# ucsdmanorlab/PSSR2

Measured on AMD Instinct MI355X. Metric: HR tiles/sec (512^2 4xSR) train, higher is better.
Workload: dtype bf16

## Files before the change

include/pssr_mi355.h:

```cpp
#ifndef PSSR_MI355_H
#define PSSR_MI355_H

#include <stdint.h>

#ifdef __cplusplus
extern "C" {
#endif

typedef void* pssr_stream_t;

enum { PSSR_F32 = 0, PSSR_BF16 = 1, PSSR_F16 = 2 };

enum {
    PSSR_OK = 0,
    PSSR_ERR_ARG = -1,
    PSSR_ERR_LAUNCH = -2,
    PSSR_ERR_UNSUPPORTED = -3
};

int pssr_abi_version(void);
const char* pssr_last_error(void);

int pssr_pack_conv_weight(const float* w_oihw, void* packed, int cout, int cin, int ks,
                          int ci_begin, int ci_count, int mode, const int32_t* n_perm,
// ... 25 lines not shown
#define PSSR_STAT_STRIPES 32
#define PSSR_STAT_ROWS (2 * PSSR_STAT_STRIPES)

enum {
    PSSR_FLAG_RELU = 1,
    PSSR_FLAG_STATS = 2,
    PSSR_FLAG_HEADQ = 8,
    PSSR_FLAG_AFFINE = 4,
    PSSR_FLAG_SOLO = 32,
    PSSR_FLAG_SHUF2 = 16
};

typedef struct pssr_conv_desc {
    int32_t dtype;
    int32_t n, h, w;
    const void* in0; int32_t in0_cstride, in0_coff, cin0, taps0;
    const void* w0;
    const void* in1; int32_t in1_cstride, in1_coff, cin1, taps1;
    const void* w1;
    int32_t prologue;
    const float* pro_scale;
    const float* pro_shift;
    void* out; int32_t out_cstride, out_coff, cout, n_pad;
    const float* bias;
    int32_t epilogue, flags;
    const void* aux; int32_t aux_cstride, aux_coff;
    const float* aux_scale; const float* aux_shift;
    const float* aux_mean; const float* aux_invstd;
    double* stats;
    int32_t in0_blk, out_blk, aux_blk;
    float out_scale, out_shift;
    void* workspace; int64_t workspace_bytes;
    const float* head_w; float* head_q;
} pssr_conv_desc;

int pssr_conv2d(const pssr_conv_desc* desc, pssr_stream_t stream);
int64_t pssr_conv2d_workspace_bytes(const pssr_conv_desc* desc);
int pssr_conv2d_pipeline_mode(int mode);

int pssr_set_option(const char* name, int value);
int pssr_get_option(const char* name);

typedef struct pssr_wgrad_desc {
    int32_t dtype;
    int32_t n, h, w;
    const void* dy; int32_t dy_cstride, dy_coff, dy_blk, cout;
    const void* in; int32_t in_cstride, in_coff, in_blk, cin_pad;
    int32_t taps;
    int32_t prologue; const float* pro_scale; const float* pro_shift;
    float* dw;
    int32_t dw_parts;
} pssr_wgrad_desc;

int pssr_conv2d_wgrad(const pssr_wgrad_desc* desc, pssr_stream_t stream);
int pssr_conv2d_wgrad_parts(const pssr_wgrad_desc* desc);



int pssr_channel_stats_nchw(const float* x, int n, int c, int64_t hw, float pre_scale, float pre_shift,
                            double* stats, pssr_stream_t stream);

int pssr_bn_finalize(const double* stats, double count, const float* gamma, const float* beta, float eps,
                     float momentum, float* running_mean, float* running_var, float* scale, float* shift,
                     float* mean, float* invstd, int c, pssr_stream_t stream);
int pssr_bn_eval_affine(const float* gamma, const float* beta, const float* running_mean,
                        const float* running_var, float eps, float* scale, float* shift, int c,
                        pssr_stream_t stream);
int pssr_bn_relu_apply(const void* y, int y_cs, int y_co, const float* scale, const float* shift, void* a, int a_cs,
                       int a_co, int64_t npix, int c, int dtype, pssr_stream_t stream);
// ... 270 lines not shown
```

pssr2_amd/_lib.py:

```python
from __future__ import annotations

import ctypes as C
import os
from pathlib import Path

_LIB_PATH = Path(__file__).resolve().parent / "libpssr_mi355.so"
_lib = None

F32, BF16, F16 = 0, 1, 2
PRO_NONE, PRO_BN_RELU, PRO_GELU = 0, 1, 2
EPI_STORE, EPI_TAIL, EPI_DGRAD_MASK, EPI_FINAL, EPI_DGRAD_GELU, EPI_HEADQ = 0, 1, 2, 3, 4, 5
FLAG_RELU, FLAG_STATS, FLAG_AFFINE, FLAG_HEADQ, FLAG_SHUF2, FLAG_SOLO = 1, 2, 4, 8, 16, 32

c_void_p, c_int, c_i64, c_float = C.c_void_p, C.c_int, C.c_int64, C.c_float


class ConvDesc(C.Structure):
    _fields_ = [
        ("dtype", C.c_int32), ("n", C.c_int32), ("h", C.c_int32), ("w", C.c_int32),
        ("in0", c_void_p), ("in0_cstride", C.c_int32), ("in0_coff", C.c_int32), ("cin0", C.c_int32), ("taps0", C.c_int32),
        ("w0", c_void_p),
        ("in1", c_void_p), ("in1_cstride", C.c_int32), ("in1_coff", C.c_int32), ("cin1", C.c_int32), ("taps1", C.c_int32),
        ("w1", c_void_p),
        ("prologue", C.c_int32), ("pro_scale", c_void_p), ("pro_shift", c_void_p),
        ("out", c_void_p), ("out_cstride", C.c_int32), ("out_coff", C.c_int32), ("cout", C.c_int32), ("n_pad", C.c_int32),
        ("bias", c_void_p),
        ("epilogue", C.c_int32), ("flags", C.c_int32),
        ("aux", c_void_p), ("aux_cstride", C.c_int32), ("aux_coff", C.c_int32),
        ("aux_scale", c_void_p), ("aux_shift", c_void_p), ("aux_mean", c_void_p), ("aux_invstd", c_void_p),
        ("stats", c_void_p),
        ("in0_blk", C.c_int32), ("out_blk", C.c_int32), ("aux_blk", C.c_int32),
        ("out_scale", C.c_float), ("out_shift", C.c_float),
        ("workspace", c_void_p), ("workspace_bytes", C.c_int64),
        ("head_w", c_void_p), ("head_q", c_void_p),
    ]


class WgradDesc(C.Structure):
    _fields_ = [
        ("dtype", C.c_int32), ("n", C.c_int32), ("h", C.c_int32), ("w", C.c_int32),
        ("dy", c_void_p), ("dy_cstride", C.c_int32), ("dy_coff", C.c_int32), ("dy_blk", C.c_int32), ("cout", C.c_int32),
        ("in_", c_void_p), ("in_cstride", C.c_int32), ("in_coff", C.c_int32), ("in_blk", C.c_int32), ("cin_pad", C.c_int32),
        ("taps", C.c_int32),
        ("prologue", C.c_int32), ("pro_scale", c_void_p), ("pro_shift", c_void_p),
        ("dw", c_void_p), ("dw_parts", C.c_int32),
    ]


class GatherItem(C.Structure):
    _fields_ = [("src", C.c_void_p), ("sh", C.c_int), ("sw", C.c_int), ("rot", C.c_int), ("flip_axis", C.c_int)]


class SheetDesc(C.Structure):
    _fields_ = [("base", C.c_void_p), ("frames", C.c_int), ("h", C.c_int), ("w", C.c_int), ("reserved", C.c_int)]


class WindowItem(C.Structure):
    _fields_ = [("sheet", C.c_int), ("frame0", C.c_int), ("y0", C.c_int), ("x0", C.c_int), ("rot", C.c_int), ("flip_axis", C.c_int)]


class CollagePanel(C.Structure):
    _fields_ = [("src", C.c_void_p), ("image_stride", C.c_int64), ("row_pitch", C.c_int32), ("src_h", C.c_int32), ("src_w", C.c_int32),
                ("is_f32", C.c_int32), ("yi", C.c_void_p), ("xi", C.c_void_p)]


COPY_BATCH_MAX = 16

# ... 64 lines not shown
```

pssr2_amd/csrc/conv_igemm.hip:

```cpp
#include "conv_igemm_args.h"

using pssr_conv::ConvArgs;

extern "C" int pssr_conv2d_pipeline_mode(int mode) {
    (void)mode;
    return 0;
}

static int conv2d_entry(const pssr_conv_desc* d, pssr_stream_t stream, long* query_ws);

#ifdef PSSR_V3_STAMPS
static unsigned* g_stamp_buf = nullptr;
extern "C" void pssr_debug_stamp_buffer(void* p) { g_stamp_buf = (unsigned*)p; }
#endif

extern "C" int pssr_conv2d(const pssr_conv_desc* d, pssr_stream_t stream) { return conv2d_entry(d, stream, nullptr); }

extern "C" int64_t pssr_conv2d_workspace_bytes(const pssr_conv_desc* d) {
    long bytes = 0;
    const int rc = conv2d_entry(d, nullptr, &bytes);
    return rc != PSSR_OK ? (int64_t)rc : (int64_t)bytes;
}

static int conv2d_entry(const pssr_conv_desc* d, pssr_stream_t stream, long* query_ws) {
    PSSR_CHECK(d != nullptr, PSSR_ERR_ARG, "conv2d: null desc");
    PSSR_CHECK(d->dtype == PSSR_F32 || d->dtype == PSSR_BF16 || d->dtype == PSSR_F16, PSSR_ERR_ARG, "conv2d: bad dtype %d", d->dtype);
    const int kch = d->dtype == PSSR_F32 ? 8 : 16;
    const int esz = d->dtype == PSSR_F32 ? 4 : 2;
    PSSR_CHECK(d->n > 0 && d->h > 0 && d->w > 0, PSSR_ERR_ARG, "conv2d: bad shape %dx%dx%d", d->n, d->h, d->w);
    PSSR_CHECK(query_ws || (d->in0 && d->w0 && d->out), PSSR_ERR_ARG, "conv2d: null pointer");
    PSSR_CHECK(d->cin0 > 0 && d->cin0 % kch == 0, PSSR_ERR_ARG, "conv2d: cin0=%d must be a positive multiple of %d", d->cin0, kch);
    PSSR_CHECK(d->taps0 == 9 || d->taps0 == 1, PSSR_ERR_ARG, "conv2d: taps0=%d", d->taps0);
    PSSR_CHECK((d->in0_cstride * esz) % 16 == 0 && (d->in0_coff * esz) % 16 == 0, PSSR_ERR_ARG, "conv2d: in0 stride/offset not 16-byte aligned");
    PSSR_CHECK(d->in0_coff + d->cin0 <= d->in0_cstride, PSSR_ERR_ARG, "conv2d: in0 slice exceeds stride");
    if (d->cin1) {
        PSSR_CHECK(d->in1 && d->w1 && d->cin1 % kch == 0 && d->taps1 == 1, PSSR_ERR_ARG, "conv2d: source 1 must be a 1x1 (or flat-K) source");
        PSSR_CHECK((d->in1_cstride * esz) % 16 == 0 && (d->in1_coff * esz) % 16 == 0 && d->in1_coff + d->cin1 <= d->in1_cstride, PSSR_ERR_ARG, "conv2d: in1 stride/offset");
    }
    if (d->epilogue == PSSR_EPI_FINAL) {
        PSSR_CHECK(d->cout > 0 && d->cout <= 32 && (d->flags & ~PSSR_FLAG_SOLO) == 0, PSSR_ERR_ARG, "conv2d: EPI_FINAL needs 0 < cout <= 32 and no flags");
    } else {
        PSSR_CHECK(d->cout > 0 && d->cout % 4 == 0, PSSR_ERR_ARG, "conv2d: cout=%d must be a positive multiple of 4", d->cout);
        PSSR_CHECK(d->out_coff % 4 == 0 && d->out_cstride % 4 == 0 &&
                   d->out_coff + ((d->flags & PSSR_FLAG_SHUF2) ? d->cout / 4 : d->cout) <= d->out_cstride, PSSR_ERR_ARG, "conv2d: out stride/offset");
    }
    PSSR_CHECK(d->n_pad % 128 == 0 && d->n_pad >= d->cout, PSSR_ERR_ARG, "conv2d: n_pad=%d", d->n_pad);
    PSSR_CHECK(d->prologue >= 0 && d->prologue <= PSSR_PRO_GELU, PSSR_ERR_ARG, "conv2d: prologue=%d", d->prologue);
    PSSR_CHECK(d->prologue != PSSR_PRO_BN_RELU || (d->pro_scale && d->pro_shift), PSSR_ERR_ARG, "conv2d: prologue needs scale/shift");
    PSSR_CHECK(d->epilogue >= 0 && d->epilogue <= 5, PSSR_ERR_ARG, "conv2d: epilogue=%d", d->epilogue);
    if (d->flags & PSSR_FLAG_HEADQ)
        PSSR_CHECK(d->epilogue == PSSR_EPI_STORE && !(d->flags & (PSSR_FLAG_STATS | PSSR_FLAG_AFFINE)) && (d->flags & PSSR_FLAG_RELU), PSSR_ERR_ARG,
                   "conv2d: FLAG_HEADQ goes with EPI_STORE | FLAG_RELU only");
    if (d->epilogue == PSSR_EPI_HEADQ || (d->flags & PSSR_FLAG_HEADQ)) {
        PSSR_CHECK(query_ws || (d->head_w && d->head_q), PSSR_ERR_ARG, "conv2d: EPI_HEADQ needs head_w / head_q");
        PSSR_CHECK(esz == 2 && d->cout == 1024 && d->taps0 == 9 && d->w >= 16 && d->h >= 16 && d->prologue != PSSR_PRO_GELU && !(d->flags & PSSR_FLAG_STATS),
                   PSSR_ERR_UNSUPPORTED, "conv2d: EPI_HEADQ needs 16-bit storage, a 3x3 source, cout = 16 x 64 (4 x upscaling) and at least 16x16 pixels");
    }
    PSSR_CHECK(d->in0_blk >= 0 && d->out_blk >= 0 && d->aux_blk >= 0 && d->in0_blk <= 3 && d->out_blk <= 3 && d->aux_blk <= 3, PSSR_ERR_ARG, "conv2d: blocked order");
    {
        const int mb = d->in0_blk > d->out_blk ? (d->in0_blk > d->aux_blk ? d->in0_blk : d->aux_blk) : (d->out_blk > d->aux_blk ? d->out_blk : d->aux_blk);
        PSSR_CHECK(d->h % (1 << mb) == 0 && d->w % (1 << mb) == 0, PSSR_ERR_ARG, "conv2d: blocked order needs H,W multiples of r");
    }
    if (d->epilogue == PSSR_EPI_TAIL || d->epilogue == PSSR_EPI_DGRAD_MASK) {
        PSSR_CHECK(d->aux && d->aux_scale && d->aux_shift && d->aux_coff % 4 == 0 && d->aux_cstride % 4 == 0, PSSR_ERR_ARG, "conv2d: epilogue needs aux tensor");
    }
    if (d->epilogue == PSSR_EPI_DGRAD_GELU)
        PSSR_CHECK(d->aux && d->aux_coff % 4 == 0 && d->aux_cstride % 4 == 0, PSSR_ERR_ARG, "conv2d: GELU backward needs the pre-activation as aux");
    if (d->flags & PSSR_FLAG_SHUF2) {
        PSSR_CHECK(d->epilogue == PSSR_EPI_STORE && !(d->flags & (PSSR_FLAG_STATS | PSSR_FLAG_HEADQ)) && d->out_blk == 0, PSSR_ERR_ARG,
                   "conv2d: FLAG_SHUF2 goes with EPI_STORE, without statistics, tap planes or a blocked output order");
        PSSR_CHECK(esz == 2 && d->cout % 32 == 0 && d->out_coff % 8 == 0 && d->out_cstride % 8 == 0 && pssr_tunables().conv_epi8, PSSR_ERR_UNSUPPORTED,
                   "conv2d: FLAG_SHUF2 needs 16-bit storage, cout a multiple of 32 and 8-channel aligned outputs");
    }
    if (d->flags & PSSR_FLAG_AFFINE) {
        PSSR_CHECK(d->epilogue == PSSR_EPI_STORE && !(d->flags & PSSR_FLAG_STATS) && d->aux_scale && d->aux_shift, PSSR_ERR_ARG,
                   "conv2d: FLAG_AFFINE needs EPI_STORE without statistics and aux_scale / aux_shift");
        PSSR_CHECK(esz == 2 && d->cout % 8 == 0 && d->out_coff % 8 == 0 && d->out_cstride % 8 == 0 && pssr_tunables().conv_epi8, PSSR_ERR_UNSUPPORTED,
                   "conv2d: FLAG_AFFINE needs 16-bit storage and 8-channel aligned outputs");
    }
    if (d->flags & PSSR_FLAG_STATS) {
        PSSR_CHECK(d->stats != nullptr, PSSR_ERR_ARG, "conv2d: stats buffer missing");
        PSSR_CHECK(d->epilogue != PSSR_EPI_DGRAD_MASK || (d->aux_mean && d->aux_invstd), PSSR_ERR_ARG, "conv2d: mask stats need mean/invstd");
        PSSR_CHECK(d->epilogue != PSSR_EPI_TAIL, PSSR_ERR_ARG, "conv2d: no stats on tail");
    }
    ConvArgs a;
    a.N = d->n; a.H = d->h; a.W = d->w;
    a.in[0] = d->in0; a.in_cs[0] = d->in0_cstride; a.in_co[0] = d->in0_coff; a.nchunks[0] = d->cin0 / kch; a.taps[0] = d->taps0; a.w[0] = d->w0;
    a.in[1] = d->in1; a.in_cs[1] = d->in1_cstride; a.in_co[1] = d->in1_coff; a.nchunks[1] = d->cin1 ? d->cin1 / kch : 0; a.taps[1] = d->cin1 ? d->taps1 : 1; a.w[1] = d->w1;
    a.prologue = d->prologue; a.pro_scale = d->pro_scale; a.pro_shift = d->pro_shift;
    a.out = d->out; a.out_cs = d->out_cstride; a.out_co = d->out_coff; a.cout = d->cout; a.n_pad = d->n_pad;
    a.bias = d->bias; a.epi = d->epilogue; a.flags = d->flags;
    a.aux = d->aux; a.aux_cs = d->aux_cstride; a.aux_co = d->aux_coff;
    a.aux_scale = d->aux_scale; a.aux_shift = d->aux_shift; a.aux_mean = d->aux_mean; a.aux_invstd = d->aux_invstd;
    a.stats = d->stats;
    a.in0_blk = d->in0_blk; a.out_blk = d->out_blk; a.aux_blk = d->aux_blk;
    a.out_scale = d->out_scale; a.out_shift = d->out_shift;
    const bool headq = a.epi == PSSR_EPI_HEADQ || (a.flags & PSSR_FLAG_HEADQ);
    a.head_w = headq ? d->head_w : nullptr;
    a.head_q = headq ? d->head_q : nullptr;
    a.tiles_x = a.tiles_y = a.tiles_n = 0;
    a.epi8 = esz == 2 && d->epilogue != PSSR_EPI_FINAL && d->cout % 8 == 0 && d->out_coff % 8 == 0 && d->out_cstride % 8 == 0 &&
             (d->epilogue == PSSR_EPI_STORE || d->epilogue == PSSR_EPI_HEADQ || (d->aux_coff % 8 == 0 && d->aux_cstride % 8 == 0));
    if (!pssr_tunables().conv_epi8) a.epi8 = 0;
    a.dbg = pssr_tunables().igemm_dbg;
    a.stamps = nullptr;
#ifdef PSSR_V3_STAMPS
    a.stamps = g_stamp_buf;
#endif
    long ws_query = 0;
    if (query_ws) { a.ksplit = -1; a.ws = (float*)&ws_query; }
    else { a.ws = (float*)d->workspace; a.ksplit = d->workspace ? (int)(d->workspace_bytes / 1024) : 0; }
    hipStream_t s = (hipStream_t)stream;
    const int rc = d->dtype == PSSR_BF16 ? pssr_conv::launch_bf16(a, s) : d->dtype == PSSR_F16 ? pssr_conv::launch_f16(a, s) : pssr_conv::launch_f32(a, s);
    if (query_ws) *query_ws = ws_query;
    return rc;
}
```

pssr2_amd/csrc/conv_igemm_args.h:

```cpp
#pragma once
#include "common.h"
#include "tunables.h"

namespace pssr_conv {

struct ConvArgs {
    int N, H, W;
    int tiles_x, tiles_y, tiles_n;
    const void* in[2]; int in_cs[2]; int in_co[2]; int nchunks[2]; int taps[2]; const void* w[2];
    int prologue; const float* pro_scale; const float* pro_shift;
    void* out; int out_cs, out_co, cout, n_pad;
    const float* bias;
    int epi, flags;
    const void* aux; int aux_cs, aux_co;
    const float* aux_scale; const float* aux_shift; const float* aux_mean; const float* aux_invstd;
    double* stats;
    int in0_blk, out_blk, aux_blk;
    float out_scale, out_shift;
    int epi8;
    unsigned* stamps;
    int dbg;
    int ksplit; float* ws;
    const float* head_w; float* head_q;
};

int launch_bf16(const ConvArgs& a, hipStream_t s);
int launch_f16(const ConvArgs& a, hipStream_t s);
int launch_f32(const ConvArgs& a, hipStream_t s);

}
```

pssr2_amd/csrc/conv_igemm_impl.h:

```cpp
#pragma once
#include <type_traits>

#include "conv_igemm_args.h"

using pssr_conv::ConvArgs;

namespace {



constexpr int PRO_LDS_MAX = 4096 * 8;

template <int GEO> struct Geo;
template <> struct Geo<0> { static constexpr int TWL = 4, THL = 3; };
template <> struct Geo<1> { static constexpr int TWL = 3, THL = 3; };
template <> struct Geo<2> { static constexpr int TWL = 2, THL = 2; };
template <> struct Geo<3> { static constexpr int TWL = 1, THL = 1; };
template <> struct Geo<4> { static constexpr int TWL = 0, THL = 0; };
template <> struct Geo<5> { static constexpr int TWL = 4, THL = 4; };

template <int BN, int GEO> struct Cfg {
    static constexpr int TWL = Geo<GEO>::TWL, THL = Geo<GEO>::THL;
    static constexpr bool BIG = GEO == 5;
    static_assert(!BIG || BN == 64, "the 256-pixel tile is built for 64 output channels");
// ... 124 lines not shown
            }
            if (p.epi == PSSR_EPI_STORE && (p.flags & PSSR_FLAG_STATS)) {
#pragma unroll
                for (int e = 0; e < 4; ++e) { const float g = X::round(v[e]); s1[e] += g; s2[e] += g * g; }
            }
            store4(outp + pix * p.out_cs + p.out_co + n_base, v);
        }
    }
    if (p.flags & PSSR_FLAG_STATS) {
#pragma unroll
        for (int off = 32; off >= CG; off >>= 1)
#pragma unroll
            for (int e = 0; e < 4; ++e) { s1[e] += __shfl_xor(s1[e], off); s2[e] += __shfl_xor(s2[e], off); }
        if (lane < CG) {
#pragma unroll
            for (int e = 0; e < 4; ++e) {
                Red[(wave * BN + lane * 4 + e) * 2 + 0] = s1[e];
                Red[(wave * BN + lane * 4 + e) * 2 + 1] = s2[e];
            }
        }
        __syncthreads();
        if (tid < BN && n0 + tid < p.cout) {
            float t1 = 0, t2 = 0;
#pragma unroll
            for (int w = 0; w < 4; ++w) { t1 += Red[(w * BN + tid) * 2]; t2 += Red[(w * BN + tid) * 2 + 1]; }
            double* st = p.stats + (long)(blockIdx.x % PSSR_STAT_STRIPES) * 2 * p.cout;
            const long lo = (long)PSSR_STAT_STRIPES * 2 * p.cout;
            stat_add(st + n0 + tid, lo, t1);
            stat_add(st + p.cout + n0 + tid, lo, t2);
        }
    }
}

template <typename T, int BN, class C, int EPI, bool STATS, bool TR = false, bool AFF = false>
__device__ __forceinline__ void conv_epilogue8(const ConvArgs& p, f32x16 (&acc)[C::MI][C::NJ], char* smem, int tid, int x0, int y0, int img0, int n0) {
    static_assert(!AFF || (EPI == PSSR_EPI_STORE && !STATS), "FLAG_AFFINE: EPI_STORE without statistics");
    using X = TT<T>;
    static_assert(sizeof(T) == 2, "8-channel pieces are 16 bytes of a 16-bit type");
    const int lane = tid & 63, wave = tid >> 6;
    const int wm = wave / C::WN, wn = wave % C::WN;
    const int h = lane >> 5, r = lane & 31;
    float* Es = (float*)smem;
    float* Red = (float*)(smem + C::E_BYTES);
    constexpr int CG = BN / 8, RP = 256 / CG;
    constexpr int EP = TR ? BN + 4 : BN;
    constexpr int ROWS = C::WM * 32, PASSES = ROWS / RP;
    static_assert(PASSES >= 1 && ROWS % RP == 0, "pass geometry");
    int wcol[C::NJ];
#pragma unroll
    for (int nj = 0; nj < C::NJ; ++nj) {
        const int col = wn * C::NJ * 32 + nj * 32 + r;
        wcol[nj] = ((col >> 2) & 1) * (BN / 2) + ((col >> 3) << 2) + (col & 3);
    }
    auto es_write = [&](int mi) {
        if constexpr (TR) {
#pragma unroll
            for (int nj = 0; nj < C::NJ; ++nj)
#pragma unroll
                for (int q = 0; q < 4; ++q) {
                    const int c = (wn * C::NJ + nj) * 4 + q;
                    *(float4*)(Es + (wm * 32 + r) * EP + h * (BN / 2) + 4 * c) =
                        make_float4(acc[mi][nj][4 * q], acc[mi][nj][4 * q + 1], acc[mi][nj][4 * q + 2], acc[mi][nj][4 * q + 3]);
                }
        } else {
#pragma unroll
            for (int nj = 0; nj < C::NJ; ++nj)
// ... 78 lines not shown
#pragma unroll
                for (int e = 0; e < 8; ++e) {
                    if (EPI == PSSR_EPI_DGRAD_GELU) asm volatile("v_add_f32 %0, %0, %1" : "+v"(s1[e]) : "v"(g[e]));
                    else s1[e] += g[e];
                    s2[e] += g[e] * (EPI == PSSR_EPI_STORE ? g[e] : a[e]);
                }
            }
            const long opix = shuf ? ((long)gi * 2 * p.H + 2 * gy + shuf_i) * (2 * p.W) + 2 * gx + shuf_j : pix_index(gi, gy, gx, p.H, p.W, p.out_blk);
            *(u32x4*)(outp + opix * p.out_cs) = packed;
        }
    }
    if (STATS) {
#pragma unroll
        for (int off = 32; off >= CG; off >>= 1)
#pragma unroll
            for (int e = 0; e < 8; ++e) { s1[e] += __shfl_xor(s1[e], off); s2[e] += __shfl_xor(s2[e], off); }
        if (lane < CG) {
#pragma unroll
            for (int e = 0; e < 8; ++e) {
                Red[(wave * BN + lane * 8 + e) * 2 + 0] = s1[e];
                Red[(wave * BN + lane * 8 + e) * 2 + 1] = s2[e];
            }
        }
        __syncthreads();
        if (tid < BN && n0 + tid < p.cout) {
            float t1 = 0, t2 = 0;
#pragma unroll
            for (int w = 0; w < 4; ++w) { t1 += Red[(w * BN + tid) * 2]; t2 += Red[(w * BN + tid) * 2 + 1]; }
            double* st = p.stats + (long)(blockIdx.x % PSSR_STAT_STRIPES) * 2 * p.cout;
            const long lo = (long)PSSR_STAT_STRIPES * 2 * p.cout;
            stat_add(st + n0 + tid, lo, t1);
            stat_add(st + p.cout + n0 + tid, lo, t2);
        }
    }
}

constexpr int HEADQ_LDS = (64 * 9 + 128) * 4;
__device__ __forceinline__ void conv_headq_stage(const ConvArgs& p, float* hq, int tid, int n0) {
    for (int i = tid; i < 64 * 9; i += 256) hq[i] = p.head_w[i];
    if (tid < 128) hq[576 + tid] = (p.bias && n0 + tid < p.cout) ? p.bias[n0 + tid] : 0.f;
}

template <typename T, class C>
__device__ __forceinline__ void conv_headq_epilogue(const ConvArgs& p, f32x16 (&acc)[C::MI][C::NJ], const float* hq, char* smem, int tid, int x0, int y0, int img0,
                                                    int n0) {
    using X = TT<T>;
    static_assert(sizeof(T) == 2 && C::NJ == 2 && C::MI == 4, "conv_v3 tiles of 128 channels");
    const int lane = tid & 63, wave = tid >> 6;
    const int wm = wave / C::WN, wn = wave % C::WN;
    const int h = lane >> 5, r = lane & 31;
    const int cbase = n0 + wn * 64;
    const int sub = cbase >> 6;
    float bias[2][16];
    u32x4 wa[2][2];
#pragma unroll
    for (int nj = 0; nj < 2; ++nj) {
#pragma unroll
        for (int e = 0; e < 16; ++e) bias[nj][e] = hq[576 + wn * 64 + nj * 32 + (e & 3) + 8 * (e >> 2) + 4 * h];
#pragma unroll
        for (int ks = 0; ks < 2; ++ks) {
            float wv[8];
#pragma unroll
            for (int i = 0; i < 8; ++i) {
                const int e = 8 * ks + i;
                const int c = nj * 32 + (e & 3) + 8 * (e >> 2) + 4 * h;
                wv[i] = r < 9 ? hq[c * 9 + r] : 0.f;
// ... 677 lines not shown
```

pssr2_amd/engine.py:

```python
from __future__ import annotations

import os
from types import SimpleNamespace

import torch

from . import _lib as L
from . import atrous as A
from . import ops

BN_EPS, BN_MOMENTUM = 1e-5, 0.1


def _blocked_order(r: int):
    if r < 1:
        raise ValueError(f"upscaling factor must be a positive integer, got scale={r}")
    l = r.bit_length() - 1
    return (l, False) if (1 << l) == r else (0, True)


_NO_MATERIALISE = os.environ.get("PSSR_MATERIALISE", "0") != "1"
_XCOL_SIDE = os.environ.get("PSSR_XCOL_SIDE", "0") == "1"
_FUSE_DOUT = os.environ.get("PSSR_FUSE_DOUT", "1") != "0"
_OVERWRITE_GRADS = os.environ.get("PSSR_OVERWRITE_GRADS", "1") != "0"
_EVAL_SHUF = os.environ.get("PSSR_EVAL_SHUF", "1") != "0"
_EVAL_AFFINE = os.environ.get("PSSR_EVAL_AFFINE", "1") != "0"
_HEAD_FUSE = os.environ.get("PSSR_HEAD_FUSE", "1") != "0"

FWD, DGRAD = dict(mode=0), dict(mode=1)
FWD_FLAT, DGRAD_FLAT = dict(mode=2), dict(mode=3)
FWD_CENTER, DGRAD_CENTER = dict(mode=2, center=True), dict(mode=3, center=True)


class _Arena:

    def __init__(self):
        self.req = []

    def take(self, n):
        self.req.append(n)
        return len(self.req) - 1

    def build(self, dtype, device):
        offs, tot = [], 0
        for n in self.req:
            offs.append(tot)
            tot += (n + 3) // 4 * 4
        self.buf = torch.zeros(max(tot, 4), dtype=dtype, device=device)
        self.views = [self.buf[o:o + n] for o, n in zip(offs, self.req)]
        return self


class _BNState:
    def __init__(self, c, f32: _Arena, f64: _Arena):
        self.c = c
        self.i32 = [f32.take(c) for _ in range(7)]
# ... 494 lines not shown
        ev, fn = d
        with torch.cuda.stream(self._side):
            self._side.wait_event(ev)
            fn()
        self._fwd_side = True

    def _folded_last(self, module, st, conv, code, perm=None):
        cache = self._fold_cache
        rp = module.respass
        key = (self._wepoch[0], conv.weight._version, conv.bias._version, rp.bias._version, st.eval_key)
        ck = (id(conv), code, perm is not None)
        ent = cache.get(ck)
        if ent is None or ent[0] != key:
            with torch.no_grad():
                wf = conv.weight.detach() * st.scale.view(-1, 1, 1, 1)
                bf = torch.addcmul(st.shift, conv.bias.detach(), st.scale).add_(rp.bias.detach())
                if perm is not None:
                    wf, bf = wf[perm], bf[perm]
                wf = wf.contiguous()
            pw = ops.pack_conv_weight(wf, code, mode=0, out=ent[1] if ent is not None else None)
            if ent is not None:
                bf = ent[2].copy_(bf)
            ent = cache[ck] = (key, pw, bf)
        return ent[1], ent[2]

    def _shuf_perm(self, c, device):
        cache = self._shuf_perms
        if (c, device) not in cache:
            idx = torch.arange(c, device=device)
            perm = (idx % (c // 4)) * 4 + idx // (c // 4)
            cache[(c, device)] = (perm, perm.to(torch.int32))
        return cache[(c, device)]

    def _block_forward(self, p, blk, module, src, cin, first, dst, dst_coff, train, shuf=None):
        if blk.a is not None:
            A.ablock_forward(self, blk.a, module, p.xin if first else src, 0, p.n, p.code, dst, dst_coff, train)
            return
        n = p.n
        hh, ww = p.dims[blk.level]
        count = float(n * hh * ww)
        nl = len(blk.y)
        rp = module.respass
        fwd_in, fwd_rp = (FWD_FLAT, FWD_CENTER) if first else (FWD, FWD)
        if not train and p.code != L.F32 and _EVAL_AFFINE and blk.c % 8 == 0:
            for k in range(nl):
                conv, bn = module.conv[3 * k], module.conv[3 * k + 1]
                self._bn_forward(blk.bn[k], bn, count, False)
                spec, inp, icn = (fwd_in, src, cin) if k == 0 else (FWD, blk.y[k - 1], blk.c)
                if k < nl - 1:
                    pw = self._pw(conv, "fwd", p.code, **spec)
                    ops.conv2d(inp, icn, pw, blk.y[k], blk.c, n=n, h=hh, w=ww, bias=conv.bias, flags=L.FLAG_RELU | L.FLAG_AFFINE,
                               aux_scale=blk.bn[k].scale, aux_shift=blk.bn[k].shift)
                    continue
                pwr = self._pw(rp, "fwd", p.code, **fwd_rp)
                if spec is FWD:
                    if shuf is not None and _EVAL_SHUF and blk.c % 32 == 0 and not first:
                        perm_l, perm_i = self._shuf_perm(blk.c, inp.device)
                        pwf, bf = self._folded_last(module, blk.bn[k], conv, p.code, perm_l)
                        pwr = self._pw(rp, "fwd_shuf", p.code, mode=0, n_perm=perm_i)
                        ops.conv2d(inp, icn, pwf, shuf, blk.c, n=n, h=hh, w=ww, out_coff=0, bias=bf, x1=src, cin1=cin, w1=pwr,
                                   flags=L.FLAG_RELU | L.FLAG_SHUF2)
                        return True
                    pwf, bf = self._folded_last(module, blk.bn[k], conv, p.code)
                    ops.conv2d(inp, icn, pwf, dst, blk.c, n=n, h=hh, w=ww, out_coff=dst_coff, bias=bf, x1=src, cin1=cin, w1=pwr,
                               flags=L.FLAG_RELU)
                    return
                pw = self._pw(conv, "fwd", p.code, **spec)
                ops.conv2d(inp, icn, pw, blk.y[k], blk.c, n=n, h=hh, w=ww, bias=conv.bias)
            nl = 0
        for k in range(nl):
            conv = module.conv[3 * k]
            bn = module.conv[3 * k + 1]
            if k == 0:
                pw = self._pw(conv, "fwd", p.code, **fwd_in)
                ops.conv2d(src, cin, pw, blk.y[0], blk.c, n=n, h=hh, w=ww, bias=conv.bias,
                           flags=L.FLAG_STATS if train else 0, stats=blk.bn[0].stats if train else None)
            else:
                pw = self._pw(conv, "fwd", p.code, **FWD)
                prev = blk.bn[k - 1]
                ops.conv2d(blk.y[k - 1], blk.c, pw, blk.y[k], blk.c, n=n, h=hh, w=ww, bias=conv.bias,
                           pro_scale=prev.scale, pro_shift=prev.shift,
                           flags=L.FLAG_STATS if train else 0, stats=blk.bn[k].stats if train else None)
                self._flush_fwd()
            self._bn_forward(blk.bn[k], bn, count, train)
            if train and k < nl - 1 and self._will_backward and self._materialise_ok(p, blk.c):
                self._materialise(p, blk, k)
        pw = self._pw(rp, "fwd", p.code, **fwd_rp)
        last = blk.bn[-1]
        ops.conv2d(src, cin, pw, dst, blk.c, n=n, h=hh, w=ww, out_coff=dst_coff, bias=rp.bias, epilogue=L.EPI_TAIL,
                   aux=blk.y[-1], aux_scale=last.scale, aux_shift=last.shift)

    def _forward_begin(self, x, train):
        m = self.model
        if not x.is_cuda:
            raise RuntimeError(f"pssr2_amd.{type(m).__name__} runs on an MI355X (HIP) device only; there is no CPU fallback")
        x = x.contiguous().float()
        self._structure(x.device)
        n, c, h, w = x.shape
        if c != self.cin:
            raise ValueError(f"expected {self.cin} input channels, got {c}")
        dt = self.storage_dtype(train)
        code = ops.dtype_code(dt)
        self._check_supported(code, h, w, train)
        p = self._plan(n, h, w, dt, x.device)
        self._repack_all(code)
        if train:
            p.f64.buf.zero_()
            self._count_batches()
        if self.atrous:
            p.bn_in.scale.fill_(1.0), p.bn_in.shift.zero_()
            if p.xin is not None:
                ops.input_plain(x, p.xin, code)
        else:
            if train:
                ops.channel_stats_nchw(x, p.bn_in.stats, 1 / 128, -1.0)
            self._bn_forward(p.bn_in, m.norm, float(n * h * w), train)
        ops.input_im2col(x, p.xcol, p.bn_in.scale, p.bn_in.shift, code)
        return x, p

    def forward(self, x, train):
        m = self.model
        x, p = self._forward_begin(x, train)
        n, code = p.n, p.code
        Lv, hid = self.L, self.hidden
        for i in range(Lv):
            blk = p.enc[i]
            src, cin = (p.xcol, self.xc) if i == 0 else (p.pooled[i - 1], ops.pad_to(hid[i - 1], 16))
            if i < Lv - 1:
                dst, off = p.cat[i], hid[i + 1] // 4
            else:
                dst, off = blk.out, 0
            shuffled = self._block_forward(p, blk, m.encoder[i], src, cin, i == 0, dst, off, train,
                                           shuf=p.cat[Lv - 2] if (i == Lv - 1 and Lv > 1 and p.epool is None and not train) else None)
            if i < Lv - 1:
                ops.maxpool2(dst, p.pooled[i], n, *p.dims[i], hid[i], code, in_coff=off)
        deep = p.enc[Lv - 1].out
        if p.epool is not None:
            A.psp_forward(self, p.epool, m.encoder_pool, deep, 0, n, code, p.epool_out, 0, train)
            deep = p.epool_out
        for l in range(Lv - 2, -1, -1):
            prev = deep if l == Lv - 2 else p.dec[l + 1].out
            if not shuffled:
                ops.pixel_shuffle(prev, p.cat[l], n, *p.dims[l + 1], hid[l + 1] // 4, 2, code)
            blk = p.dec[l]
            shuffled = self._block_forward(p, blk, m.decoder[Lv - 2 - l], p.cat[l], p.cat[l].shape[-1], False, blk.out, 0, train,
                                           shuf=p.cat[l - 1] if (l > 0 and not train) else None)
        feat = p.dec[0].out if Lv > 1 else deep
        if p.rpool is not None:
            A.psp_forward(self, p.rpool, m.reconstruction_pool, feat, 0, n, code, p.rpool_out, 0, train)
            feat = p.rpool_out
        out = self._head_forward(p, feat, x, train)
        self._flush_fwd()
        self.saved = (p, x) if train else None
        return out

    def _head_forward(self, p, feat, x, train=True):
        rec = self.model.reconstruction
        n, h, w, code, h0, r = p.n, p.h, p.w, p.code, self.h0, self.r
        pw0, pw1 = self._pw_pre("fwd0", code), self._pw_pre("fwd1", code)
        p.pre_bias = rec.pre.bias.detach()[self.pre_perm_long].contiguous()
        out = torch.empty(n, self.cout, h * r, w * r, dtype=torch.float32, device=x.device)
        if _HEAD_FUSE and ops.head_q_supported(code, h0, self.cout, r, h, w):
            if p.head_q is None:
                p.head_q = torch.empty(9, r * r, n, h, w, dtype=torch.float32, device=x.device)
            if train:
                ops.conv2d(feat, h0, pw0, p.pre, r * r * h0, n=n, h=h, w=w, bias=p.pre_bias, x1=p.xcol, cin1=self.xc,
                           w1=pw1, flags=L.FLAG_RELU | L.FLAG_HEADQ, head_w=rec.conv.weight, head_q=p.head_q)
            else:
                ops.conv2d(feat, h0, pw0, p.head_q, r * r * h0, n=n, h=h, w=w, bias=p.pre_bias, x1=p.xcol, cin1=self.xc,
                           w1=pw1, epilogue=L.EPI_HEADQ, head_w=rec.conv.weight, head_q=p.head_q)
            ops.head_q_gather(p.head_q, rec.conv.bias, out, n, h, w, 128.0, 128.0)
            return out
        ops.conv2d(feat, h0, pw0, p.pre, r * r * h0, n=n, h=h, w=w, bias=p.pre_bias, x1=p.xcol, cin1=self.xc, w1=pw1, flags=L.FLAG_RELU)
        pre_hr = self._pre_hr(p)
        if self.explicit_shuffle:
            ops.pixel_shuffle(p.pre, pre_hr, n, h, w, h0, r, code)
        if ops.head_conv_supported(code, h0, self.cout):
            ops.head_conv_fwd(pre_hr, self.blk, rec.conv.weight, rec.conv.bias, out, n, h * r, w * r, h0, self.cout, 128.0, 128.0, code)
        else:
# ... 276 lines not shown
```

pssr2_amd/ops.py:

```python
from __future__ import annotations

import ctypes as C

import torch

from . import _lib as L

TORCH_DTYPE = {L.F32: torch.float32, L.BF16: torch.bfloat16, L.F16: torch.float16}


def dtype_code(dt: torch.dtype) -> int:
    if dt == torch.float32:
        return L.F32
    if dt == torch.bfloat16:
        return L.BF16
    if dt == torch.float16:
        return L.F16
    raise ValueError(f"unsupported compute dtype {dt}; use torch.float32, torch.bfloat16 or torch.float16")


def pad_to(v: int, m: int) -> int:
    return (v + m - 1) // m * m


class PackedWeight:
    __slots__ = ("data", "taps", "k_pad", "n_pad", "dtype")

    def __init__(self, data, taps, k_pad, n_pad, dtype):
        self.data, self.taps, self.k_pad, self.n_pad, self.dtype = data, taps, k_pad, n_pad, dtype


def pack_conv_weight(w: torch.Tensor, dtype: int, mode: int = 0, ci_begin: int = 0, ci_count: int | None = None,
                     n_perm: torch.Tensor | None = None, out: PackedWeight | None = None) -> PackedWeight:
    assert w.is_cuda and w.dtype == torch.float32 and w.is_contiguous() and w.dim() == 4
    cout, cin, ks, _ = w.shape
    ci_count = cin - ci_begin if ci_count is None else ci_count
    s2dk = ks * ks * pad_to(cin, 16)
    gk = ci_count if mode == 0 else cout if mode in (1, 3, 5) else s2dk if mode == 4 else ci_count * ks * ks
    gn = ci_count if mode == 1 else ci_count * ks * ks if mode == 3 else s2dk if mode == 5 else cout
    taps = 1 if mode >= 2 else ks * ks
    k_pad, n_pad = pad_to(gk, 16), pad_to(gn, 128)
    if out is None:
        nbytes = L.lib().pssr_packed_weight_bytes(taps, k_pad, n_pad, dtype)
        out = PackedWeight(torch.empty(nbytes, dtype=torch.uint8, device=w.device), taps, k_pad, n_pad, dtype)
    L.check(L.lib().pssr_pack_conv_weight(L.ptr(w), L.ptr(out.data), cout, cin, ks, ci_begin, ci_count, mode,
                                          L.ptr(n_perm), k_pad, n_pad, dtype, L.stream_ptr()), "pssr_pack_conv_weight")
    return out


SOLO = [False]


def conv2d(x, cin0, w0: PackedWeight, out, cout, *, n, h, w, in0_coff=0, out_coff=0, bias=None,
           x1=None, cin1=0, w1: PackedWeight | None = None, in1_coff=0,
           pro_scale=None, pro_shift=None, epilogue=L.EPI_STORE, flags=0,
           aux=None, aux_coff=0, aux_scale=None, aux_shift=None, aux_mean=None, aux_invstd=None, stats=None,
           in0_blk=0, out_blk=0, aux_blk=0, out_scale=1.0, out_shift=0.0, gelu_in=False, head_w=None, head_q=None):
    d = L.ConvDesc()
    d.dtype = w0.dtype
    d.n, d.h, d.w = n, h, w
    d.in0, d.in0_cstride, d.in0_coff, d.cin0, d.taps0, d.w0 = L.ptr(x), x.shape[-1], in0_coff, cin0, w0.taps, L.ptr(w0.data)
    if w1 is not None:
        d.in1, d.in1_cstride, d.in1_coff, d.cin1, d.taps1, d.w1 = L.ptr(x1), x1.shape[-1], in1_coff, cin1, w1.taps, L.ptr(w1.data)
        assert w1.n_pad == w0.n_pad and w1.dtype == w0.dtype
    d.prologue = L.PRO_GELU if gelu_in else L.PRO_BN_RELU if pro_scale is not None else L.PRO_NONE
    d.pro_scale, d.pro_shift = L.ptr(pro_scale), L.ptr(pro_shift)
    d.out, d.out_cstride, d.out_coff, d.cout, d.n_pad = L.ptr(out), out.shape[-1], out_coff, cout, w0.n_pad
    d.bias = L.ptr(bias)
    d.epilogue, d.flags = epilogue, flags | (L.FLAG_SOLO if SOLO[0] else 0)
    if aux is not None:
        d.aux, d.aux_cstride, d.aux_coff = L.ptr(aux), aux.shape[-1], aux_coff
    d.aux_scale, d.aux_shift, d.aux_mean, d.aux_invstd = L.ptr(aux_scale), L.ptr(aux_shift), L.ptr(aux_mean), L.ptr(aux_invstd)
    d.stats = L.ptr(stats)
    d.in0_blk, d.out_blk, d.aux_blk, d.out_scale, d.out_shift = in0_blk, out_blk, aux_blk, out_scale, out_shift
    if epilogue == L.EPI_FINAL:
        d.out_cstride, d.out_coff = cout, 0
    if epilogue == L.EPI_HEADQ:
        d.out_cstride, d.out_coff = cout, 0
    if epilogue == L.EPI_HEADQ or flags & L.FLAG_HEADQ:
        d.head_w, d.head_q = L.ptr(head_w), L.ptr(head_q)
    ws_bytes = L.lib().pssr_conv2d_workspace_bytes(C.byref(d))
    if ws_bytes > 0:
        ws = torch.empty(ws_bytes, dtype=torch.uint8, device=out.device)
        d.workspace, d.workspace_bytes = L.ptr(ws), ws_bytes
    L.check(L.lib().pssr_conv2d(C.byref(d), L.stream_ptr()), "pssr_conv2d")
    return out


def _wgrad_desc(dy, cout, x, cin_pad, taps, *, n, h, w, dtype, dy_coff=0, in_coff=0, dy_blk=0, in_blk=0, pro_scale=None, pro_shift=None,
                gelu_in=False):
    d = L.WgradDesc()
    d.dtype, d.n, d.h, d.w = dtype, n, h, w
    d.dy, d.dy_cstride, d.dy_coff, d.dy_blk, d.cout = L.ptr(dy), dy.shape[-1], dy_coff, dy_blk, cout
    d.in_, d.in_cstride, d.in_coff, d.in_blk, d.cin_pad = L.ptr(x), x.shape[-1], in_coff, in_blk, cin_pad
    d.taps = taps
    d.prologue = L.PRO_GELU if gelu_in else L.PRO_BN_RELU if pro_scale is not None else L.PRO_NONE
    d.pro_scale, d.pro_shift = L.ptr(pro_scale), L.ptr(pro_shift)
    return d


def conv2d_wgrad(dy, cout, x, cin_pad, taps, dw, **kw):
    d = _wgrad_desc(dy, cout, x, cin_pad, taps, **kw)
    d.dw, d.dw_parts = L.ptr(dw), 0
    L.check(L.lib().pssr_conv2d_wgrad(C.byref(d), L.stream_ptr()), "pssr_conv2d_wgrad")
    return dw


def conv2d_wgrad_parts(dy, cout, x, cin_pad, taps, **kw):
    d = _wgrad_desc(dy, cout, x, cin_pad, taps, **kw)
    parts = L.lib().pssr_conv2d_wgrad_parts(C.byref(d))
    if parts <= 0:
        L.check(parts if parts < 0 else -1, "pssr_conv2d_wgrad_parts")
    dw = torch.empty(parts, cout, taps, cin_pad, dtype=torch.float32, device=dy.device)
    d.dw, d.dw_parts = L.ptr(dw), parts
    L.check(L.lib().pssr_conv2d_wgrad(C.byref(d), L.stream_ptr()), "pssr_conv2d_wgrad")
    return dw


def unpack_conv_wgrad(dw_packed, dw_oihw, *, mode=0, ci_begin=0, ci_count=None, n_perm=None, k_pad, accumulate=False):
# ... 763 lines not shown
```

Baseline: 2371.

## Fuse maxpool and pixel-shuffle into block tail conv epilogue

Adds pool_out and shuf_out targets to the conv descriptor so that the tail conv of each UNet block can write a 2x2 max-pooled copy or a pixel-shuffled copy of its output tile straight from the epilogue. This removes the separate maxpool2 and pixel_shuffle kernel launches during training, which used to run only in eval for the shuffle case. The epilogue re-reads the tile it just stored in global memory after a __syncthreads, so the launches and full-tensor passes are traded for extra in-kernel memory traffic. There is also an extra ctypes descriptor build and validity check per call.

```diff
diff --git a/include/pssr_mi355.h b/include/pssr_mi355.h
--- a/include/pssr_mi355.h
+++ b/include/pssr_mi355.h
@@ -81,9 +81,12 @@
     float out_scale, out_shift;
     void* workspace; int64_t workspace_bytes;
     const float* head_w; float* head_q;
+    void* pool_out; int32_t pool_cstride, pool_coff;
+    void* shuf_out; int32_t shuf_cstride, shuf_coff;
 } pssr_conv_desc;
 
 int pssr_conv2d(const pssr_conv_desc* desc, pssr_stream_t stream);
+int pssr_conv2d_post_ok(const pssr_conv_desc* desc);
 int64_t pssr_conv2d_workspace_bytes(const pssr_conv_desc* desc);
 int pssr_conv2d_pipeline_mode(int mode);
 
diff --git a/pssr2_amd/_lib.py b/pssr2_amd/_lib.py
--- a/pssr2_amd/_lib.py
+++ b/pssr2_amd/_lib.py
@@ -33,6 +33,8 @@
         ("out_scale", C.c_float), ("out_shift", C.c_float),
         ("workspace", c_void_p), ("workspace_bytes", C.c_int64),
         ("head_w", c_void_p), ("head_q", c_void_p),
+        ("pool_out", c_void_p), ("pool_cstride", C.c_int32), ("pool_coff", C.c_int32),
+        ("shuf_out", c_void_p), ("shuf_cstride", C.c_int32), ("shuf_coff", C.c_int32),
     ]
 
 
diff --git a/pssr2_amd/csrc/conv_igemm.hip b/pssr2_amd/csrc/conv_igemm.hip
--- a/pssr2_amd/csrc/conv_igemm.hip
+++ b/pssr2_amd/csrc/conv_igemm.hip
@@ -20,6 +20,29 @@
     long bytes = 0;
     const int rc = conv2d_entry(d, nullptr, &bytes);
     return rc != PSSR_OK ? (int64_t)rc : (int64_t)bytes;
+}
+
+static const char* conv2d_post_reject(const pssr_conv_desc* d) {
+    if (d->dtype != PSSR_BF16 && d->dtype != PSSR_F16) return "16-bit storage only";
+    const bool store = d->epilogue == PSSR_EPI_STORE && !(d->flags & (PSSR_FLAG_STATS | PSSR_FLAG_SHUF2 | PSSR_FLAG_HEADQ));
+    if (d->epilogue != PSSR_EPI_TAIL && !store) return "EPI_TAIL, or EPI_STORE without statistics, FLAG_SHUF2 and tap planes";
+    if (d->out_blk != 0) return "no blocked output order";
+    if (d->cout <= 0 || d->cout % 8 || d->out_coff % 8 || d->out_cstride % 8 || !pssr_tunables().conv_epi8) return "8-channel aligned outputs";
+    if (d->epilogue == PSSR_EPI_TAIL && (d->aux_coff % 8 || d->aux_cstride % 8)) return "8-channel aligned aux";
+    if (d->w < 2 || d->h < 1) return "at least two pixels per row";
+    if (d->pool_out) {
+        if (d->h % 2 || d->w % 2) return "pool_out needs even h and w";
+        if (d->pool_cstride % 8 || d->pool_coff % 8 || d->pool_coff < 0 || d->pool_coff + d->cout > d->pool_cstride) return "pool_out stride / offset";
+    }
+    if (d->shuf_out) {
+        if (d->cout % 32) return "shuf_out needs cout a multiple of 32";
+        if (d->shuf_cstride % 8 || d->shuf_coff % 8 || d->shuf_coff < 0 || d->shuf_coff + d->cout / 4 > d->shuf_cstride) return "shuf_out stride / offset";
+    }
+    return nullptr;
+}
+
+extern "C" int pssr_conv2d_post_ok(const pssr_conv_desc* d) {
+    return d != nullptr && (d->pool_out || d->shuf_out) && conv2d_post_reject(d) == nullptr;
 }
 
 static int conv2d_entry(const pssr_conv_desc* d, pssr_stream_t stream, long* query_ws) {
@@ -83,7 +106,13 @@
         PSSR_CHECK(d->epilogue != PSSR_EPI_DGRAD_MASK || (d->aux_mean && d->aux_invstd), PSSR_ERR_ARG, "conv2d: mask stats need mean/invstd");
         PSSR_CHECK(d->epilogue != PSSR_EPI_TAIL, PSSR_ERR_ARG, "conv2d: no stats on tail");
     }
+    if (d->pool_out || d->shuf_out) {
+        const char* why = conv2d_post_reject(d);
+        PSSR_CHECK(why == nullptr, PSSR_ERR_ARG, "conv2d: pool_out / shuf_out: %s", why);
+    }
     ConvArgs a;
+    a.pool_out = d->pool_out; a.pool_cs = d->pool_cstride; a.pool_co = d->pool_coff;
+    a.shuf_out = d->shuf_out; a.shuf_cs = d->shuf_cstride; a.shuf_co = d->shuf_coff;
     a.N = d->n; a.H = d->h; a.W = d->w;
     a.in[0] = d->in0; a.in_cs[0] = d->in0_cstride; a.in_co[0] = d->in0_coff; a.nchunks[0] = d->cin0 / kch; a.taps[0] = d->taps0; a.w[0] = d->w0;
     a.in[1] = d->in1; a.in_cs[1] = d->in1_cstride; a.in_co[1] = d->in1_coff; a.nchunks[1] = d->cin1 ? d->cin1 / kch : 0; a.taps[1] = d->cin1 ? d->taps1 : 1; a.w[1] = d->w1;
diff --git a/pssr2_amd/csrc/conv_igemm_args.h b/pssr2_amd/csrc/conv_igemm_args.h
--- a/pssr2_amd/csrc/conv_igemm_args.h
+++ b/pssr2_amd/csrc/conv_igemm_args.h
@@ -22,6 +22,8 @@
     int dbg;
     int ksplit; float* ws;
     const float* head_w; float* head_q;
+    void* pool_out; int pool_cs, pool_co;
+    void* shuf_out; int shuf_cs, shuf_co;
 };
 
 int launch_bf16(const ConvArgs& a, hipStream_t s);
diff --git a/pssr2_amd/csrc/conv_igemm_impl.h b/pssr2_amd/csrc/conv_igemm_impl.h
--- a/pssr2_amd/csrc/conv_igemm_impl.h
+++ b/pssr2_amd/csrc/conv_igemm_impl.h
@@ -180,6 +180,72 @@
     }
 }
 
+template <typename T, int BN, class C>
+__device__ __forceinline__ void conv_tile_post(const ConvArgs& p, int tid, int x0, int y0, int img0, int n0) {
+    static_assert(sizeof(T) == 2, "16-bit storage");
+    if constexpr (C::TW >= 2 && C::TH >= 2) {
+        __syncthreads();
+        const T* const outp = (const T*)p.out + p.out_co;
+        if (p.pool_out) {
+            constexpr int CG = BN / 8, WX = C::TW / 2, WY = C::TH / 2, ITEMS = WX * WY * C::NI * CG;
+            T* const dst = (T*)p.pool_out + p.pool_co;
+            const int ho = p.H >> 1, wo = p.W >> 1;
+            const long down = (long)p.W * p.out_cs;
+#pragma unroll 1
+            for (int i = tid; i < ITEMS; i += 256) {
+                const int c0 = n0 + (i % CG) * 8;
+                int wd = i / CG;
+                const int wx = wd % WX; wd /= WX;
+                const int wy = wd % WY;
+                const int gi = img0 + wd / WY, gy = y0 + 2 * wy, gx = x0 + 2 * wx;
+                if (!(c0 < p.cout && gi < p.N && gy < p.H && gx < p.W)) continue;
+                const T* s = outp + (((long)gi * p.H + gy) * p.W + gx) * p.out_cs + c0;
+                float a[8], b[8], cc[8], d[8], m[8];
+                load4(s, a); load4(s + 4, a + 4);
+                load4(s + p.out_cs, b); load4(s + p.out_cs + 4, b + 4);
+                load4(s + down, cc); load4(s + down + 4, cc + 4);
+                load4(s + down + p.out_cs, d); load4(s + down + p.out_cs + 4, d + 4);
+#pragma unroll
+                for (int e = 0; e < 8; ++e) m[e] = fmaxf(fmaxf(a[e], b[e]), fmaxf(cc[e], d[e]));
+                T* q = dst + (((long)gi * ho + (gy >> 1)) * wo + (gx >> 1)) * p.pool_cs + c0;
+                store4(q, m); store4(q + 4, m + 4);
+            }
+        }
+        if (p.shuf_out) {
+            constexpr int G = BN / 32, ITEMS = C::TW * C::TH * C::NI * G;
+            const unsigned short* const src = (const unsigned short*)outp;
+            unsigned short* const dst = (unsigned short*)p.shuf_out + p.shuf_co;
+#pragma unroll 1
+            for (int i = tid; i < ITEMS; i += 256) {
+                const int c0 = n0 + (i % G) * 32;
+                int m = i / G;
+                const int tx = m % C::TW; m /= C::TW;
+                const int ty = m % C::TH;
+                const int gi = img0 + m / C::TH, gy = y0 + ty, gx = x0 + tx;
+                if (!(c0 < p.cout && gi < p.N && gy < p.H && gx < p.W)) continue;
+                const unsigned short* s = src + (((long)gi * p.H + gy) * p.W + gx) * p.out_cs + c0;
+                unsigned w[16];
+#pragma unroll
+                for (int q = 0; q < 4; ++q) {
+                    const u32x4 t = *(const u32x4*)(s + 8 * q);
+                    w[4 * q] = t[0]; w[4 * q + 1] = t[1]; w[4 * q + 2] = t[2]; w[4 * q + 3] = t[3];
+                }
+#pragma unroll
+                for (int k = 0; k < 4; ++k) {
+                    u32x4 v;
+#pragma unroll
+                    for (int j = 0; j < 4; ++j) {
+                        const unsigned lo = w[4 * j + (k >> 1)], hi = w[4 * j + 2 + (k >> 1)];
+                        v[j] = (k & 1) ? ((lo >> 16) | (hi & 0xffff0000u)) : ((lo & 0xffffu) | (hi << 16));
+                    }
+                    const long phi = ((long)gi * 2 * p.H + 2 * gy + (k >> 1)) * (2L * p.W) + 2 * gx + (k & 1);
+                    *(u32x4*)(dst + phi * p.shuf_cs + (c0 >> 2)) = v;
+                }
+            }
+        }
+    }
+}
+
 template <typename T, int BN, class C, int EPI, bool STATS, bool TR = false, bool AFF = false>
 __device__ __forceinline__ void conv_epilogue8(const ConvArgs& p, f32x16 (&acc)[C::MI][C::NJ], char* smem, int tid, int x0, int y0, int img0, int n0) {
     static_assert(!AFF || (EPI == PSSR_EPI_STORE && !STATS), "FLAG_AFFINE: EPI_STORE without statistics");
@@ -324,6 +390,9 @@
             stat_add(st + n0 + tid, lo, t1);
             stat_add(st + p.cout + n0 + tid, lo, t2);
         }
+    }
+    if constexpr (EPI == PSSR_EPI_TAIL || (EPI == PSSR_EPI_STORE && !STATS)) {
+        if (p.pool_out || p.shuf_out) conv_tile_post<T, BN, C>(p, tid, x0, y0, img0, n0);
     }
 }
 
diff --git a/pssr2_amd/engine.py b/pssr2_amd/engine.py
--- a/pssr2_amd/engine.py
+++ b/pssr2_amd/engine.py
@@ -22,6 +22,7 @@
 _NO_MATERIALISE = os.environ.get("PSSR_MATERIALISE", "0") != "1"
 _XCOL_SIDE = os.environ.get("PSSR_XCOL_SIDE", "0") == "1"
 _FUSE_DOUT = os.environ.get("PSSR_FUSE_DOUT", "1") != "0"
+_FUSE_TAIL = os.environ.get("PSSR_FUSE_TAIL", "1") != "0"
 _OVERWRITE_GRADS = os.environ.get("PSSR_OVERWRITE_GRADS", "1") != "0"
 _EVAL_SHUF = os.environ.get("PSSR_EVAL_SHUF", "1") != "0"
 _EVAL_AFFINE = os.environ.get("PSSR_EVAL_AFFINE", "1") != "0"
@@ -582,7 +583,7 @@
             cache[(c, device)] = (perm, perm.to(torch.int32))
         return cache[(c, device)]
 
-    def _block_forward(self, p, blk, module, src, cin, first, dst, dst_coff, train, shuf=None):
+    def _block_forward(self, p, blk, module, src, cin, first, dst, dst_coff, train, shuf=None, pool=None):
         if blk.a is not None:
             A.ablock_forward(self, blk.a, module, p.xin if first else src, 0, p.n, p.code, dst, dst_coff, train)
             return
@@ -612,11 +613,11 @@
                                    flags=L.FLAG_RELU | L.FLAG_SHUF2)
                         return True
                     pwf, bf = self._folded_last(module, blk.bn[k], conv, p.code)
-                    ops.conv2d(inp, icn, pwf, dst, blk.c, n=n, h=hh, w=ww, out_coff=dst_coff, bias=bf, x1=src, cin1=cin, w1=pwr,
-                               flags=L.FLAG_RELU)
-                    return
+                    return self._conv_post(pool, None, inp, icn, pwf, dst, blk.c, n=n, h=hh, w=ww, out_coff=dst_coff, bias=bf, x1=src, cin1=cin,
+                                           w1=pwr, flags=L.FLAG_RELU)
                 pw = self._pw(conv, "fwd", p.code, **spec)
                 ops.conv2d(inp, icn, pw, blk.y[k], blk.c, n=n, h=hh, w=ww, bias=conv.bias)
+                pool = shuf = None
             nl = 0
         for k in range(nl):
             conv = module.conv[3 * k]
@@ -637,8 +638,17 @@
                 self._materialise(p, blk, k)
         pw = self._pw(rp, "fwd", p.code, **fwd_rp)
         last = blk.bn[-1]
-        ops.conv2d(src, cin, pw, dst, blk.c, n=n, h=hh, w=ww, out_coff=dst_coff, bias=rp.bias, epilogue=L.EPI_TAIL,
-                   aux=blk.y[-1], aux_scale=last.scale, aux_shift=last.shift)
+        return self._conv_post(pool, shuf, src, cin, pw, dst, blk.c, n=n, h=hh, w=ww, out_coff=dst_coff, bias=rp.bias, epilogue=L.EPI_TAIL,
+                               aux=blk.y[-1], aux_scale=last.scale, aux_shift=last.shift)
+
+    @staticmethod
+    def _conv_post(pool, shuf, *args, **kw):
+        post = {"pool_out": pool} if pool is not None else {"shuf_out": shuf} if shuf is not None else None
+        if post is not None and _FUSE_TAIL and ops.conv2d_post_ok(*args, **kw, **post):
+            ops.conv2d(*args, **kw, **post)
+            return True
+        ops.conv2d(*args, **kw)
+        return None
 
     def _forward_begin(self, x, train):
         m = self.model
@@ -680,10 +690,12 @@
                 dst, off = p.cat[i], hid[i + 1] // 4
             else:
                 dst, off = blk.out, 0
-            shuffled = self._block_forward(p, blk, m.encoder[i], src, cin, i == 0, dst, off, train,
-                                           shuf=p.cat[Lv - 2] if (i == Lv - 1 and Lv > 1 and p.epool is None and not train) else None)
-            if i < Lv - 1:
+            wrote = self._block_forward(p, blk, m.encoder[i], src, cin, i == 0, dst, off, train,
+                                        shuf=p.cat[Lv - 2] if (i == Lv - 1 and Lv > 1 and p.epool is None) else None,
+                                        pool=p.pooled[i] if i < Lv - 1 else None)
+            if i < Lv - 1 and not wrote:
                 ops.maxpool2(dst, p.pooled[i], n, *p.dims[i], hid[i], code, in_coff=off)
+        shuffled = wrote
         deep = p.enc[Lv - 1].out
         if p.epool is not None:
             A.psp_forward(self, p.epool, m.encoder_pool, deep, 0, n, code, p.epool_out, 0, train)
@@ -694,7 +706,7 @@
                 ops.pixel_shuffle(prev, p.cat[l], n, *p.dims[l + 1], hid[l + 1] // 4, 2, code)
             blk = p.dec[l]
             shuffled = self._block_forward(p, blk, m.decoder[Lv - 2 - l], p.cat[l], p.cat[l].shape[-1], False, blk.out, 0, train,
-                                           shuf=p.cat[l - 1] if (l > 0 and not train) else None)
+                                           shuf=p.cat[l - 1] if l > 0 else None)
         feat = p.dec[0].out if Lv > 1 else deep
         if p.rpool is not None:
             A.psp_forward(self, p.rpool, m.reconstruction_pool, feat, 0, n, code, p.rpool_out, 0, train)
diff --git a/pssr2_amd/ops.py b/pssr2_amd/ops.py
--- a/pssr2_amd/ops.py
+++ b/pssr2_amd/ops.py
@@ -51,11 +51,12 @@
 SOLO = [False]
 
 
-def conv2d(x, cin0, w0: PackedWeight, out, cout, *, n, h, w, in0_coff=0, out_coff=0, bias=None,
-           x1=None, cin1=0, w1: PackedWeight | None = None, in1_coff=0,
-           pro_scale=None, pro_shift=None, epilogue=L.EPI_STORE, flags=0,
-           aux=None, aux_coff=0, aux_scale=None, aux_shift=None, aux_mean=None, aux_invstd=None, stats=None,
-           in0_blk=0, out_blk=0, aux_blk=0, out_scale=1.0, out_shift=0.0, gelu_in=False, head_w=None, head_q=None):
+def _conv_desc(x, cin0, w0: PackedWeight, out, cout, *, n, h, w, in0_coff=0, out_coff=0, bias=None,
+               x1=None, cin1=0, w1: PackedWeight | None = None, in1_coff=0,
+               pro_scale=None, pro_shift=None, epilogue=L.EPI_STORE, flags=0,
+               aux=None, aux_coff=0, aux_scale=None, aux_shift=None, aux_mean=None, aux_invstd=None, stats=None,
+               in0_blk=0, out_blk=0, aux_blk=0, out_scale=1.0, out_shift=0.0, gelu_in=False, head_w=None, head_q=None,
+               pool_out=None, pool_coff=0, shuf_out=None, shuf_coff=0):
     d = L.ConvDesc()
     d.dtype = w0.dtype
     d.n, d.h, d.w = n, h, w
@@ -79,12 +80,25 @@
         d.out_cstride, d.out_coff = cout, 0
     if epilogue == L.EPI_HEADQ or flags & L.FLAG_HEADQ:
         d.head_w, d.head_q = L.ptr(head_w), L.ptr(head_q)
+    if pool_out is not None:
+        d.pool_out, d.pool_cstride, d.pool_coff = L.ptr(pool_out), pool_out.shape[-1], pool_coff
+    if shuf_out is not None:
+        d.shuf_out, d.shuf_cstride, d.shuf_coff = L.ptr(shuf_out), shuf_out.shape[-1], shuf_coff
+    return d
+
+
+def conv2d(x, cin0, w0: PackedWeight, out, cout, **kw):
+    d = _conv_desc(x, cin0, w0, out, cout, **kw)
     ws_bytes = L.lib().pssr_conv2d_workspace_bytes(C.byref(d))
     if ws_bytes > 0:
         ws = torch.empty(ws_bytes, dtype=torch.uint8, device=out.device)
         d.workspace, d.workspace_bytes = L.ptr(ws), ws_bytes
     L.check(L.lib().pssr_conv2d(C.byref(d), L.stream_ptr()), "pssr_conv2d")
     return out
+
+
+def conv2d_post_ok(x, cin0, w0: PackedWeight, out, cout, **kw) -> bool:
+    return bool(L.lib().pssr_conv2d_post_ok(C.byref(_conv_desc(x, cin0, w0, out, cout, **kw))))
 
 
 def _wgrad_desc(dy, cout, x, cin_pad, taps, *, n, h, w, dtype, dy_coff=0, in_coff=0, dy_blk=0, in_blk=0, pro_scale=None, pro_shift=None,
```

After: 2385, median of 2. No clear change (+0.6%).
